# atong01/conditional-flow-matching

Measured on NVIDIA B200. Metric: minibatch-OT couplings/sec (N=8192,d=784), higher is better.
Workload: dtype f32

## Files before the change

cfm_b200/csrc/sinkhorn_common.cuh:

```cuda
#pragma once
#include <cooperative_groups.h>

#include "common.cuh"

namespace cg = cooperative_groups;

namespace cfm {

constexpr int kSkThreads = 512;
constexpr int kSkWarps = kSkThreads / 32;
constexpr int kSkChunk = kSkWarps;
constexpr int kSkMaxKG = 4;
constexpr int kPanelCols = kSkThreads * 4 * kSkMaxKG;

struct SkParams {
  const float* M;
  int n0, n1;
  int64_t ldm;
  float reg;
  const float* cost_max;
  int normalize;
  int max_iters;
  double stop_thr;
  int check_every;
  int precise;
  double stall_tol;
  double* log_u;
  double* log_v;
  int32_t* status;
  double* err_out;
  void* u_work;
  void* v_work[2];
  void* part_m;
  void* part_s;
  double* err_ring;
  int n1p;
  int vec;
  int v_in_smem;
  float l2_resident_frac;
  int dbg_flags;
  int atomic_cols;
  int prefetch_chunks;
  int run_if;
  int timeline;
  int screen_fused;
  int screen;
  int mixed;
};

template <bool P> struct Tr;
template <> struct Tr<false> {
  using pot_t = float;
  using sum_t = float;
  __device__ static __forceinline__ float init() { return -1.0e30f; }
};
template <> struct Tr<true> {
  using pot_t = double;
  using sum_t = double;
  __device__ static __forceinline__ double init() { return -1.0e300; }
};

template <bool P> struct Xf;
template <> struct Xf<false> {
  float c2;
  __device__ __forceinline__ float operator()(float m, float p) const { return fmaf(m, c2, p); }
};
template <> struct Xf<true> {
  float reg, cmax;
  int norm;
  __device__ __forceinline__ double operator()(float m, double p) const {
    const float mn = norm ? __fdiv_rn(m, cmax) : m;
    return (double)(-__fdiv_rn(mn, reg)) + p;
  }
};
__device__ __forceinline__ float expdiff(float x, float m) { return ex2f(x - m); }
__device__ __forceinline__ double expdiff(double x, double m) { return exp(x - m); }
template <bool MIX> __device__ __forceinline__ float expd(float x, float m) { return ex2f(x - m); }
template <bool MIX> __device__ __forceinline__ double expd(double x, double m) {
  if (MIX) return (double)ex2f((float)(x - m) * kLog2e);
  return exp(x - m);
}
__device__ __forceinline__ float lse_fin(float m, float s) { return m + log2f(s); }
__device__ __forceinline__ double lse_fin(double m, double s) { return m + log(s); }
__device__ __forceinline__ float vmax(float a, float b) { return fmaxf(a, b); }
__device__ __forceinline__ double vmax(double a, double b) { return fmax(a, b); }

template <bool VEC>
__device__ __forceinline__ float4 load_cost4(const float* __restrict__ row, int j, int n1) {
  if (VEC) return ldg_stream4(row + j);
  float4 r;
  const float inf = __int_as_float(0x7f800000);
  r.x = (j + 0 < n1) ? __ldg(row + j + 0) : inf;
  r.y = (j + 1 < n1) ? __ldg(row + j + 1) : inf;
  r.z = (j + 2 < n1) ? __ldg(row + j + 2) : inf;
  r.w = (j + 3 < n1) ? __ldg(row + j + 3) : inf;
  return r;
}

template <class T> struct Vec4 { T x, y, z, w; };

template <bool SM, class T>
__device__ __forceinline__ Vec4<T> load_pot4(const T* p, int j) {
  Vec4<T> r;
  if (SM) { r.x = p[j]; r.y = p[j + 1]; r.z = p[j + 2]; r.w = p[j + 3]; }
  else { r.x = __ldcg(p + j); r.y = __ldcg(p + j + 1); r.z = __ldcg(p + j + 2); r.w = __ldcg(p + j + 3); }
  return r;
}

}
```

cfm_b200/csrc/sinkhorn_v2.cu:

```cuda
#include <stdlib.h>

#include "sinkhorn_common.cuh"

namespace cfm {


__device__ __forceinline__ uint32_t v2_smem_u32(const void* p) { return (uint32_t)__cvta_generic_to_shared(p); }
__device__ __forceinline__ void v2_mbar_init(uint64_t* bar, uint32_t count) {
  asm volatile("mbarrier.init.shared::cta.b64 [%0], %1;" ::"r"(v2_smem_u32(bar)), "r"(count));
}
__device__ __forceinline__ void v2_mbar_expect_tx(uint64_t* bar, uint32_t bytes) {
  asm volatile("mbarrier.arrive.expect_tx.shared::cta.b64 _, [%0], %1;" ::"r"(v2_smem_u32(bar)), "r"(bytes) : "memory");
}
__device__ __forceinline__ void v2_mbar_arrive(uint64_t* bar) {
  asm volatile("mbarrier.arrive.shared::cta.b64 _, [%0];" ::"r"(v2_smem_u32(bar)) : "memory");
}
__device__ __forceinline__ void v2_mbar_wait(uint64_t* bar, uint32_t parity) {
  asm volatile(
      "{\n\t"
      ".reg .pred p;\n\t"
      "WAIT_%=:\n\t"
      "mbarrier.try_wait.parity.shared::cta.b64 p, [%0], %1;\n\t"
      "@p bra DONE_%=;\n\t"
      "bra WAIT_%=;\n\t"
      "DONE_%=:\n\t"
      "}\n" ::"r"(v2_smem_u32(bar)), "r"(parity) : "memory");
}
__device__ __forceinline__ void v2_bulk_load(void* dst, const void* src, uint32_t bytes, uint64_t* bar) {
  asm volatile("cp.async.bulk.shared::cluster.global.mbarrier::complete_tx::bytes [%0], [%1], %2, [%3];"
               ::"r"(v2_smem_u32(dst)), "l"(src), "r"(bytes), "r"(v2_smem_u32(bar)) : "memory");
}
__device__ __forceinline__ void v2_bulk_load_hint(void* dst, const void* src, uint32_t bytes, uint64_t* bar,
                                                  uint64_t policy) {
  asm volatile("cp.async.bulk.shared::cluster.global.mbarrier::complete_tx::bytes.L2::cache_hint [%0], [%1], %2, [%3], %4;"
               ::"r"(v2_smem_u32(dst)), "l"(src), "r"(bytes), "r"(v2_smem_u32(bar)), "l"(policy) : "memory");
}
__device__ __forceinline__ void v2_prefetch_l2(const void* src, uint32_t bytes) {
  asm volatile("cp.async.bulk.prefetch.L2.global [%0], %1;" ::"l"(src), "r"(bytes) : "memory");
}
__device__ __forceinline__ uint64_t v2_policy_evict_last() {
  uint64_t p;
  asm volatile("createpolicy.fractional.L2::evict_last.b64 %0, 1.0;" : "=l"(p));
  return p;
}
__device__ __forceinline__ uint64_t v2_policy_evict_first() {
  uint64_t p;
  asm volatile("createpolicy.fractional.L2::evict_first.b64 %0, 1.0;" : "=l"(p));
  return p;
}
__device__ __forceinline__ void v2_grid_barrier(unsigned int* counter, unsigned int target) {
  __syncthreads();
  if (threadIdx.x == 0) {
    __threadfence();
    atomicAdd(counter, 1u);
    unsigned int seen;
    do {
      asm volatile("ld.acquire.gpu.global.u32 %0, [%1];" : "=r"(seen) : "l"(counter) : "memory");
    } while (seen < target);
    __threadfence();
  }
  __syncthreads();
}
template <int NT>
__device__ __forceinline__ void v2_consumer_barrier() { asm volatile("bar.sync 1, %0;" ::"n"(NT) : "memory"); }

template <int R>
__device__ __forceinline__ void multi_reduce(float (&v)[R], int lane) {
  static_assert(R == 1 || R == 2 || R == 4 || R == 8, "R must be a power of two <= 8");
  int off = 16;
#pragma unroll
  for (int n = R; n > 1; n >>= 1) {
    const bool upper = (lane & off) != 0;
#pragma unroll
    for (int i = 0; i < n / 2; ++i) {
      const float a = v[2 * i], b = v[2 * i + 1];
      const float send = upper ? a : b, keep = upper ? b : a;
      v[i] = keep + __shfl_xor_sync(0xffffffffu, send, off);
    }
    off >>= 1;
  }
  for (; off > 0; off >>= 1) v[0] += __shfl_xor_sync(0xffffffffu, v[0], off);
}
template <int R>
__device__ __forceinline__ int multi_row(int lane) {
  int r = 0, bit = 4;
#pragma unroll
  for (int n = R, sh = 0; n > 1; n >>= 1, ++sh, --bit) r |= ((lane >> bit) & 1) << sh;
  return r;
}

template <int NT, int KG, int R>
__global__ void __launch_bounds__(NT, 512 / NT) sinkhorn_v2_kernel(const SkParams p, const int S) {
  constexpr int kV2Consumers = NT, kV2Threads = NT, kV2Warps = NT / 32;
  constexpr bool kVSmem = KG > 4;
  extern __shared__ __align__(128) unsigned char v2_smem[];
  cg::grid_group grid = cg::this_grid();
  const int tid = threadIdx.x, lane = tid & 31, warp = tid >> 5;
  const int nblk = gridDim.x, b = blockIdx.x;
  const int n0 = p.n0, n1 = p.n1, n1p = p.n1p, ng = n1p / 4;

  if (p.run_if != 0) {
    const float cmax = p.cost_max ? __ldg(p.cost_max) : 0.f;
    const bool precise = !((p.normalize ? 1.f : cmax) / p.reg <= 64.f);
    if (precise) return;
  }

  const uint32_t stage_floats = (uint32_t)R * (uint32_t)n1p;
  float* stages = reinterpret_cast<float*>(v2_smem);
  float2* rowpart = reinterpret_cast<float2*>(stages + (size_t)S * stage_floats);
  uint64_t* full = reinterpret_cast<uint64_t*>(rowpart + 2 * R * kV2Warps);
  float* V_s = reinterpret_cast<float*>(full + 8);
  __shared__ double red[kV2Warps];

  if (tid == 0) {
    for (int s = 0; s < S; ++s) v2_mbar_init(&full[s], 1);
    asm volatile("fence.mbarrier_init.release.cluster;" ::: "memory");
  }
  __syncthreads();

  float* u_work = reinterpret_cast<float*>(p.u_work);
  float* v_work[2] = {reinterpret_cast<float*>(p.v_work[0]), reinterpret_cast<float*>(p.v_work[1])};
  float* part_m = reinterpret_cast<float*>(p.part_m);
  float* part_s = reinterpret_cast<float*>(p.part_s);

  const float cmaxv = p.cost_max ? __ldg(p.cost_max) : 1.f;
  const float c2 = -kLog2e / (p.reg * (p.normalize ? cmaxv : 1.f));
  const float loga = -log2f((float)n0), logb = -log2f((float)n1);
  const float kappa = c2 * cmaxv;
  const bool fact = (p.cost_max != nullptr) && (-kappa <= 40.f);

  const int base = n0 / nblk, rem = n0 % nblk;
  const int r_begin = b * base + min(b, rem);
  const int nrows = base + (b < rem ? 1 : 0);
  const int nchunks = (nrows + R - 1) / R;

  int c_st = 0;
  uint32_t c_par = 0;
  int p_st = 0, p_chunk = 0;
  int p_dir = 1;
  int sweep_no = 0;
  unsigned int* gbar = reinterpret_cast<unsigned int*>(p.err_ring + 4);
  unsigned int gbar_n = 0;
  auto grid_sync = [&]() { (void)gbar; (void)gbar_n; grid.sync(); };
  long long issued = 0, consumed_total = 0;
  bool gvalid[KG];
#pragma unroll
  for (int k = 0; k < KG; ++k) gvalid[k] = (tid + kV2Consumers * k) < ng;
  const int tcol = tid * 4;
  const bool full_cols = ng == kV2Consumers * KG;

  const int resident = p.l2_resident_frac > 0.f ? (int)(p.l2_resident_frac * (float)nchunks) : -1;
  const uint64_t pol_last = v2_policy_evict_last(), pol_first = v2_policy_evict_first();
  auto issue_next = [&]() {
    const int r0 = r_begin + p_chunk * R;
    const int rv = min(R, r_begin + nrows - r0);
    v2_mbar_expect_tx(&full[p_st], (uint32_t)rv * (uint32_t)n1 * 4u);
    for (int r = 0; r < rv; ++r) {
      float* dst = stages + (size_t)p_st * stage_floats + (size_t)r * n1p;
      const float* src = p.M + (int64_t)(r0 + r) * p.ldm;
      if (resident < 0) v2_bulk_load(dst, src, (uint32_t)n1 * 4u, &full[p_st]);
      else v2_bulk_load_hint(dst, src, (uint32_t)n1 * 4u, &full[p_st], p_chunk < resident ? pol_last : pol_first);
    }
    ++issued;
    p_chunk += p_dir;
    if (p_chunk == nchunks) { p_chunk = nchunks - 1; p_dir = -1; }
    else if (p_chunk < 0) { p_chunk = 0; p_dir = 1; }
    if (++p_st == S) p_st = 0;
  };
  if (tid == 0)
    for (int q = 0; q < S; ++q) issue_next();
  auto prefetch_ahead = [&]() {
    int c = p_chunk, dir = p_dir;
    for (int q = 0; q < p.prefetch_chunks; ++q) {
      if (c < 0 || c >= nchunks) break;
      if (!(resident >= 0 && c < resident)) {
        const int r0 = r_begin + c * R;
        const int rv = min(R, r_begin + nrows - r0);
        for (int r = 0; r < rv; ++r) v2_prefetch_l2(p.M + (int64_t)(r0 + r) * p.ldm, (uint32_t)n1 * 4u);
      }
      c += dir;
    }
  };

  auto sweep = [&](bool do_row, bool do_col, const float* v_cur, const float4* v_in, float vref_in,
                   unsigned long long* acc_out, const float* v_reload) {
    if (fact) {
      const float vref = do_row ? (v_in ? vref_in : __ldcg(v_cur)) : 0.f;
      const float nkap = -kappa;
      float4 V[kVSmem ? 1 : KG];
      float cs[KG][4];
#pragma unroll
      for (int k = 0; k < KG; ++k) {
        float4 vk = make_float4(0.f, 0.f, 0.f, 0.f);
        if (gvalid[k]) {
          if (do_row) {
            const float4 vv = v_in ? v_in[k]
                                   : __ldcg(reinterpret_cast<const float4*>(v_cur + tcol + kV2Consumers * 4 * k));
            vk = make_float4(ex2f(vv.x - vref), ex2f(vv.y - vref), ex2f(vv.z - vref), ex2f(vv.w - vref));
          } else {
            vk = make_float4(1.f, 1.f, 1.f, 1.f);
          }
        }
        if (kVSmem) *reinterpret_cast<float4*>(V_s + tcol + kV2Consumers * 4 * k) = vk;
        else V[k] = vk;
#pragma unroll
        for (int c = 0; c < 4; ++c) cs[k][c] = 0.f;
      }
      float uref = 0.f;
      bool have_uref = !do_row;
      for (int cc = 0; cc < nchunks; ++cc) {
        const int chunk = (sweep_no & 1) ? nchunks - 1 - cc : cc;
        const int r0 = r_begin + chunk * R;
        const int rv = min(R, r_begin + nrows - r0);
        const float* sbase = stages + (uint32_t)c_st * stage_floats + tcol;
        float2* rp = rowpart + (cc & 1) * R * kV2Warps;
        v2_mbar_wait(&full[c_st], c_par);
        float4 E[R][KG];
        if (full_cols && rv == R) {
#pragma unroll
          for (int r = 0; r < R; ++r)
#pragma unroll
            for (int k = 0; k < KG; ++k) {
              const float4 mv = *reinterpret_cast<const float4*>(sbase + r * n1p + kV2Consumers * 4 * k);
              E[r][k] = make_float4(ex2f(fmaf(mv.x, c2, nkap)), ex2f(fmaf(mv.y, c2, nkap)),
                                    ex2f(fmaf(mv.z, c2, nkap)), ex2f(fmaf(mv.w, c2, nkap)));
            }
        } else {
#pragma unroll
          for (int r = 0; r < R; ++r) {
            const float* srow = sbase + r * n1p;
#pragma unroll
            for (int k = 0; k < KG; ++k) {
              E[r][k] = make_float4(0.f, 0.f, 0.f, 0.f);
              if (gvalid[k] && r < rv) {
                const float4 mv = *reinterpret_cast<const float4*>(srow + kV2Consumers * 4 * k);
                E[r][k] = make_float4(ex2f(fmaf(mv.x, c2, nkap)), ex2f(fmaf(mv.y, c2, nkap)),
                                      ex2f(fmaf(mv.z, c2, nkap)), ex2f(fmaf(mv.w, c2, nkap)));
              }
            }
          }
        }
        if (++c_st == S) { c_st = 0; c_par ^= 1u; }
        if (do_row) {
          float sr[R];
#pragma unroll
          for (int r = 0; r < R; ++r) {
            float s = 0.f;
#pragma unroll
            for (int k = 0; k < KG; ++k) {
              const float4 vk = kVSmem ? *reinterpret_cast<const float4*>(V_s + tcol + kV2Consumers * 4 * k)
                                       : V[kVSmem ? 0 : k];
              s = fmaf(E[r][k].x, vk.x, s); s = fmaf(E[r][k].y, vk.y, s);
              s = fmaf(E[r][k].z, vk.z, s); s = fmaf(E[r][k].w, vk.w, s);
            }
            sr[r] = s;
          }
          multi_reduce<R>(sr, lane);
          if ((lane & (32 / R - 1)) == 0) rp[multi_row<R>(lane) * kV2Warps + warp] = make_float2(sr[0], 0.f);
        }
        v2_consumer_barrier<NT>();
        if (tid == 0) issue_next();
        float U[R];
        if (do_row) {
#pragma unroll
          for (int rr = 0; rr < R; rr += 2) {
            const int myrow = rr + (lane >> 4);
            float pr = ((R == 1 && lane >= 16) || (lane & 15) >= kV2Warps)
                           ? 0.f : rp[(R == 1 ? 0 : myrow) * kV2Warps + (lane & 15)].x;
#pragma unroll
            for (int o = 8; o > 0; o >>= 1) pr += __shfl_xor_sync(0xffffffffu, pr, o);
            float Srow[2];
            Srow[0] = __shfl_sync(0xffffffffu, pr, 0);
            Srow[1] = __shfl_sync(0xffffffffu, pr, 16);
#pragma unroll
            for (int h = 0; h < 2; ++h) {
              const int r = rr + h;
              if (r < R) {
                const float u2 = loga - (kappa + vref + lg2_abs(Srow[h]));
                if (!have_uref) { uref = u2; have_uref = true; }
                U[r] = r < rv ? ex2f(u2 - uref) : 0.f;
                if (warp == 0 && lane == 0 && r < rv) {
                  u_work[r0 + r] = u2;
                  p.log_u[r0 + r] = (double)u2 * kLn2d;
                }
              }
            }
          }
        } else {
#pragma unroll
          for (int r = 0; r < R; ++r) U[r] = 1.f;
        }
        if (do_col) {
#pragma unroll
          for (int r = 0; r < R; ++r)
#pragma unroll
            for (int k = 0; k < KG; ++k) {
              cs[k][0] = fmaf(E[r][k].x, U[r], cs[k][0]); cs[k][1] = fmaf(E[r][k].y, U[r], cs[k][1]);
              cs[k][2] = fmaf(E[r][k].z, U[r], cs[k][2]); cs[k][3] = fmaf(E[r][k].w, U[r], cs[k][3]);
            }
        }
      }
      consumed_total += nchunks;
      ++sweep_no;
      if (tid == 0) prefetch_ahead();
      if (do_col && acc_out != nullptr) {
        const float sh = kappa + uref - logb;
#pragma unroll
        for (int k = 0; k < KG; ++k)
          if (gvalid[k]) {
            const float4 vv = v_reload ? __ldcg(reinterpret_cast<const float4*>(v_reload + tcol + kV2Consumers * 4 * k))
                                       : make_float4(0.f, 0.f, 0.f, 0.f);
            const float vq[4] = {vv.x, vv.y, vv.z, vv.w};
            unsigned long long* dst = acc_out + tcol + kV2Consumers * 4 * k;
#pragma unroll
            for (int c = 0; c < 4; ++c) {
              const float q = cs[k][c] * ex2f(sh + vq[c]) * 4294967296.f;
              atomicAdd(dst + c, (unsigned long long)__float2ll_rn(fminf(fmaxf(q, 0.f), 4.0e18f)));
            }
          }
      } else if (do_col) {
        const float pm = kappa + uref;
#pragma unroll
        for (int k = 0; k < KG; ++k)
          if (gvalid[k]) {
            *reinterpret_cast<float4*>(part_m + (int64_t)b * n1p + tcol + kV2Consumers * 4 * k) =
                make_float4(pm, pm, pm, pm);
            *reinterpret_cast<float4*>(part_s + (int64_t)b * n1p + tcol + kV2Consumers * 4 * k) =
                make_float4(cs[k][0], cs[k][1], cs[k][2], cs[k][3]);
          }
      }
      return;
    }
    float4 vreg[KG];
    float cm[KG][4], cs[KG][4];
#pragma unroll
    for (int k = 0; k < KG; ++k) {
      vreg[k] = make_float4(0.f, 0.f, 0.f, 0.f);
      if (do_row && gvalid[k]) {
        const float* vp = v_cur + tcol + kV2Consumers * 4 * k;
        vreg[k] = make_float4(__ldcg(vp), __ldcg(vp + 1), __ldcg(vp + 2), __ldcg(vp + 3));
      }
#pragma unroll
      for (int c = 0; c < 4; ++c) { cm[k][c] = -1.0e30f; cs[k][c] = 0.f; }
    }
    const float inf = __int_as_float(0x7f800000);
    for (int cc = 0; cc < nchunks; ++cc) {
      const int chunk = (sweep_no & 1) ? nchunks - 1 - cc : cc;
      const int r0 = r_begin + chunk * R;
      const int rv = min(R, r_begin + nrows - r0);
      const float* sbase = stages + (uint32_t)c_st * stage_floats + tcol;
      float2* rp = rowpart + (cc & 1) * R * kV2Warps;
      v2_mbar_wait(&full[c_st], c_par);
      if (++c_st == S) { c_st = 0; c_par ^= 1u; }
      float u2[R];
      if (do_row) {
#pragma unroll
        for (int r = 0; r < R; ++r) {
          float x[KG][4];
          float tmax = -1.0e30f;
#pragma unroll
          for (int k = 0; k < KG; ++k) {
            float4 mv = make_float4(inf, inf, inf, inf);
            if (gvalid[k] && r < rv) mv = *reinterpret_cast<const float4*>(sbase + r * n1p + kV2Consumers * 4 * k);
            x[k][0] = fmaf(mv.x, c2, vreg[k].x); x[k][1] = fmaf(mv.y, c2, vreg[k].y);
            x[k][2] = fmaf(mv.z, c2, vreg[k].z); x[k][3] = fmaf(mv.w, c2, vreg[k].w);
            tmax = fmaxf(tmax, fmaxf(fmaxf(x[k][0], x[k][1]), fmaxf(x[k][2], x[k][3])));
          }
          const float wm = warp_max(tmax);
          float s = 0.f;
#pragma unroll
          for (int k = 0; k < KG; ++k)
            s += (ex2f(x[k][0] - wm) + ex2f(x[k][1] - wm)) + (ex2f(x[k][2] - wm) + ex2f(x[k][3] - wm));
          s = warp_sum(s);
          if (lane == 0) rp[r * kV2Warps + warp] = make_float2(wm, s);
        }
      }
      v2_consumer_barrier<NT>();
#pragma unroll
      for (int r = 0; r < R; ++r) {
        u2[r] = 0.f;
        if (do_row) {
          const float2 pr = lane < kV2Warps ? rp[r * kV2Warps + lane] : make_float2(-1.0e30f, 0.f);
          const float gm = warp_max(pr.x);
          const float gs = warp_sum(pr.y * ex2f(pr.x - gm));
          u2[r] = loga - (gm + log2f(gs));
          if (warp == 0 && lane == 0 && r < rv) {
            u_work[r0 + r] = u2[r];
            p.log_u[r0 + r] = (double)u2[r] * kLn2d;
          }
        }
      }
      if (do_col) {
#pragma unroll
        for (int r = 0; r < R; ++r) {
          if (r < rv) {
#pragma unroll
            for (int k = 0; k < KG; ++k) {
              if (gvalid[k]) {
                const float4 mv = *reinterpret_cast<const float4*>(sbase + r * n1p + kV2Consumers * 4 * k);
                const float xv[4] = {fmaf(mv.x, c2, u2[r]), fmaf(mv.y, c2, u2[r]), fmaf(mv.z, c2, u2[r]),
                                     fmaf(mv.w, c2, u2[r])};
#pragma unroll
                for (int c = 0; c < 4; ++c) {
                  if (xv[c] > cm[k][c] + 40.f) {
                    cs[k][c] *= ex2f(cm[k][c] - xv[c]);
                    cm[k][c] = xv[c];
                  }
                  cs[k][c] += ex2f(xv[c] - cm[k][c]);
                }
              }
            }
          }
        }
      }
      v2_consumer_barrier<NT>();
      if (tid == 0) issue_next();
    }
    consumed_total += nchunks;
    ++sweep_no;
    if (tid == 0) prefetch_ahead();
    if (do_col) {
#pragma unroll
      for (int k = 0; k < KG; ++k)
        if (gvalid[k]) {
          *reinterpret_cast<float4*>(part_m + (int64_t)b * n1p + tcol + kV2Consumers * 4 * k) =
              make_float4(cm[k][0], cm[k][1], cm[k][2], cm[k][3]);
          *reinterpret_cast<float4*>(part_s + (int64_t)b * n1p + tcol + kV2Consumers * 4 * k) =
              make_float4(cs[k][0], cs[k][1], cs[k][2], cs[k][3]);
        }
    }
  };

  auto combine = [&](const float* v_cur, float* v_new, bool have_cur, double* err_slot) {
    double err_local = 0.0;
    const int cpc = (n1 + nblk - 1) / nblk;
    const int c_begin = b * cpc, c_end = min(n1, c_begin + cpc);
    const int sub = tid & 7;
    for (int j0 = c_begin; j0 < c_end; j0 += (kV2Consumers >> 3)) {
      const int j = j0 + (tid >> 3);
      const bool act = j < c_end;
      float m = -1.0e30f, s = 0.f;
      if (act) {
        if (p.dbg_flags & 1) {
          for (int c0 = sub; c0 < nblk; c0 += 32) {
            float mm[4], ss[4];
#pragma unroll
            for (int q = 0; q < 4; ++q) {
              const int c = c0 + q * 8;
              if (c < nblk) {
                mm[q] = __ldcg(part_m + (int64_t)c * n1p + j);
                ss[q] = __ldcg(part_s + (int64_t)c * n1p + j);
              } else { mm[q] = -1.0e30f; ss[q] = 0.f; }
            }
            const float bm = fmaxf(fmaxf(fmaxf(mm[0], mm[1]), fmaxf(mm[2], mm[3])), m);
            float acc = s * ex2f(m - bm);
#pragma unroll
            for (int q = 0; q < 4; ++q) acc += ss[q] * ex2f(mm[q] - bm);
            s = acc; m = bm;
          }
        } else if (!(p.dbg_flags & 4) && nblk <= 152) {
          float mm[19], ss[19];
#pragma unroll
          for (int q = 0; q < 19; ++q) {
            const int c = sub + q * 8;
            if (c < nblk) {
              mm[q] = __ldcg(part_m + (int64_t)c * n1p + j);
              ss[q] = __ldcg(part_s + (int64_t)c * n1p + j);
            } else { mm[q] = -1.0e30f; ss[q] = 0.f; }
          }
          float bm = m;
#pragma unroll
          for (int q = 0; q < 19; ++q) bm = fmaxf(bm, mm[q]);
          float acc = 0.f;
#pragma unroll
          for (int q = 0; q < 19; ++q) acc += ss[q] * ex2f(mm[q] - bm);
          s = acc; m = bm;
        } else
        for (int c0 = sub; c0 < nblk; c0 += 64) {
          float mm[8], ss[8];
#pragma unroll
          for (int q = 0; q < 8; ++q) {
            const int c = c0 + q * 8;
            if (c < nblk) {
              mm[q] = __ldcg(part_m + (int64_t)c * n1p + j);
              ss[q] = __ldcg(part_s + (int64_t)c * n1p + j);
            } else { mm[q] = -1.0e30f; ss[q] = 0.f; }
          }
          float bm = m;
#pragma unroll
          for (int q = 0; q < 8; ++q) bm = fmaxf(bm, mm[q]);
          float acc = s * ex2f(m - bm);
#pragma unroll
          for (int q = 0; q < 8; ++q) acc += ss[q] * ex2f(mm[q] - bm);
          s = acc; m = bm;
        }
      }
      float gm = m;
#pragma unroll
      for (int o = 4; o > 0; o >>= 1) gm = fmaxf(gm, __shfl_xor_sync(0xffffffffu, gm, o));
      float gs = s * ex2f(m - gm);
#pragma unroll
      for (int o = 4; o > 0; o >>= 1) gs += __shfl_xor_sync(0xffffffffu, gs, o);
      if (act && sub == 0) {
        const float vn = logb - (gm + log2f(gs));
        v_new[j] = vn;
        if (have_cur) {
          const double d = ((double)__ldcg(v_cur + j) - (double)vn) * kLn2d;
          const double e = expm1(d) / (double)n1;
          err_local += e * e;
        }
      }
    }
    if (err_slot != nullptr) {
      err_local = warp_sum(err_local);
      if (lane == 0) red[warp] = err_local;
      __syncthreads();
      if (warp == 0) {
        double t = lane < kV2Warps ? red[lane] : 0.0;
        t = warp_sum(t);
        if (lane == 0) atomicAdd(err_slot, t);
      }
      __syncthreads();
    }
  };

  if (b == 0 && tid < 4) p.err_ring[tid] = 0.0;

  int cur = 0, iters = 0;
  bool converged = false;
  double err = 1.0, prev_check_err = -1.0;
  const bool single = fact && p.atomic_cols != 0;
  if (single) {
    unsigned long long* acc = reinterpret_cast<unsigned long long*>(p.part_s);
    float* vmine = part_m + (int64_t)b * n1p;
#pragma unroll
    for (int k = 0; k < KG; ++k)
      if (gvalid[k]) *reinterpret_cast<float4*>(vmine + tcol + kV2Consumers * 4 * k) = make_float4(0.f, 0.f, 0.f, 0.f);
    float vref_cur = 0.f;
    const int cpc = ((n1 + nblk - 1) / nblk + 3) & ~3;
    sweep(false, true, nullptr, nullptr, 0.f, acc, nullptr);
    grid_sync();
    for (int it = 0;; ++it) {
      const unsigned long long* tot = acc + (size_t)(it % 3) * n1p;
      {
        unsigned long long* z = acc + (size_t)((it + 2) % 3) * n1p;
        for (int j = b * cpc + tid; j < min(n1, (b + 1) * cpc); j += kV2Threads) z[j] = 0ull;
      }
      float4 vnew[KG];
      double e2 = 0.0;
      const float t0 = (float)((double)__ldcg(tot) * 2.3283064365386963e-10);
      const float vref_new = vref_cur - lg2_abs(t0);
#pragma unroll
      for (int k = 0; k < KG; ++k) {
        float4 vcur_k = make_float4(0.f, 0.f, 0.f, 0.f);
        if (gvalid[k]) vcur_k = __ldcg(reinterpret_cast<const float4*>(vmine + tcol + kV2Consumers * 4 * k));
        vnew[k] = vcur_k;
        if (gvalid[k]) {
          const ulonglong2 a = __ldcg(reinterpret_cast<const ulonglong2*>(tot + tcol + kV2Consumers * 4 * k));
          const ulonglong2 c = __ldcg(reinterpret_cast<const ulonglong2*>(tot + tcol + kV2Consumers * 4 * k + 2));
          const double td[4] = {(double)a.x * 2.3283064365386963e-10, (double)a.y * 2.3283064365386963e-10,
                                (double)c.x * 2.3283064365386963e-10, (double)c.y * 2.3283064365386963e-10};
          vnew[k] = make_float4(vcur_k.x - lg2_abs((float)td[0]), vcur_k.y - lg2_abs((float)td[1]),
                                vcur_k.z - lg2_abs((float)td[2]), vcur_k.w - lg2_abs((float)td[3]));
#pragma unroll
          for (int q = 0; q < 4; ++q) e2 += (td[q] - 1.0) * (td[q] - 1.0);
        }
      }
      if (it >= 1 && (((it - 1) % p.check_every) == 0 || (p.dbg_flags & 2))) {
        e2 = warp_sum(e2);
        if (lane == 0) red[warp] = e2;
        __syncthreads();
        double t = 0.0;
        for (int w = 0; w < kV2Warps; ++w) t += red[w];
        __syncthreads();
        err = sqrt(t) / (double)n1;
        if (((it - 1) % p.check_every) == 0) {
          if (err < p.stop_thr) { converged = true; break; }
          if (p.stall_tol > 0.0 && prev_check_err >= 0.0 && err > (1.0 - p.stall_tol) * prev_check_err &&
              err * sqrt((double)n1) < 1e-5) { converged = true; break; }
          prev_check_err = err;
        }
      }
      if (it == p.max_iters) break;
#pragma unroll
      for (int k = 0; k < KG; ++k)
        if (gvalid[k]) *reinterpret_cast<float4*>(vmine + tcol + kV2Consumers * 4 * k) = vnew[k];
      vref_cur = vref_new;
      const bool last = (it == p.max_iters - 1);
      const bool check = (it % p.check_every) == 0;
      const bool do_col = !last || check;
      sweep(true, do_col, nullptr, vnew, vref_cur, do_col ? acc + (size_t)((it + 1) % 3) * n1p : nullptr, vmine);
      iters = it + 1;
      if (!do_col) break;
      grid_sync();
    }
    if (b == 0) {
#pragma unroll
      for (int k = 0; k < KG; ++k)
        if (gvalid[k]) {
          const int j = tcol + kV2Consumers * 4 * k;
          const float4 vv = __ldcg(reinterpret_cast<const float4*>(vmine + j));
          p.log_v[j] = (double)vv.x * kLn2d; p.log_v[j + 1] = (double)vv.y * kLn2d;
          p.log_v[j + 2] = (double)vv.z * kLn2d; p.log_v[j + 3] = (double)vv.w * kLn2d;
        }
    }
  } else {
  sweep(false, true, nullptr, nullptr, 0.f, nullptr, nullptr);
  grid_sync();
  combine(nullptr, v_work[0], false, nullptr);
  grid_sync();

  for (int it = 0; it < p.max_iters; ++it) {
    const bool last = (it == p.max_iters - 1);
    const bool check = (it % p.check_every) == 0;
    const bool do_col = !last || check;
    sweep(true, do_col, v_work[cur], nullptr, 0.f, nullptr, nullptr);
    iters = it + 1;
    if (!do_col) break;
    grid_sync();
    if (b == 0 && tid == 0) p.err_ring[(it + 2) & 3] = 0.0;
    const bool want_err = check || (p.dbg_flags & 2);
    combine(v_work[cur], v_work[cur ^ 1], want_err, want_err ? &p.err_ring[it & 3] : nullptr);
    grid_sync();
    if (check) {
      err = sqrt(__ldcg(&p.err_ring[it & 3]));
      if (err < p.stop_thr) { converged = true; break; }
      if (p.stall_tol > 0.0 && prev_check_err >= 0.0 && err > (1.0 - p.stall_tol) * prev_check_err &&
          err * sqrt((double)n1) < 1e-5) { converged = true; break; }
      prev_check_err = err;
    }
    if (last) break;
    cur ^= 1;
  }
  }

  if (tid == 0) {
    for (long long q = consumed_total; q < issued; ++q) {
      v2_mbar_wait(&full[c_st], c_par);
      if (++c_st == S) { c_st = 0; c_par ^= 1u; }
    }
  }

  if (!single)
    for (int j = b * kV2Threads + tid; j < n1; j += nblk * kV2Threads)
      p.log_v[j] = (double)__ldcg(v_work[cur] + j) * kLn2d;
  if (b == 0 && tid == 0) {
    int flags = 0;
    if (!converged) flags |= CFM_FLAG_NOT_CONVERGED;
    if (!(err == err)) flags |= CFM_FLAG_NONFINITE;
    p.status[0] = flags;
    p.status[1] = iters;
    p.status[2] = 0;
    p.status[3] = fact ? (single ? 4 : 3) : 2;
    *p.err_out = err;
  }
}

template <int NT, int KG, int R>
static int v2_launch_t(SkParams& p, cudaStream_t s) {
  auto kern = sinkhorn_v2_kernel<NT, KG, R>;
  constexpr int kPerSm = 512 / NT;
  const size_t stage_bytes = (size_t)R * p.n1p * 4;
  const size_t fixed = (size_t)2 * R * (NT / 32) * sizeof(float2) + 8 * sizeof(uint64_t) + 128 +
                       (KG > 4 ? (size_t)p.n1p * 4 : 0);
  const size_t budget = (kPerSm == 1 ? 220 : 108) * 1024;
  if (budget < fixed + 2 * stage_bytes) return 1;
  int S = (int)((budget - fixed) / stage_bytes);
  if (S > 8) S = 8;
  const size_t smem = (size_t)S * stage_bytes + fixed;
  CFM_CUDA_OK(cudaFuncSetAttribute(kern, cudaFuncAttributeMaxDynamicSharedMemorySize, (int)smem));
  int per_sm = 0;
  CFM_CUDA_OK(cudaOccupancyMaxActiveBlocksPerMultiprocessor(&per_sm, kern, NT, smem));
  if (per_sm < 1) return 1;
  if (per_sm > kPerSm) per_sm = kPerSm;
  int grid = sm_count() * per_sm;
  if (grid > p.n0) grid = p.n0;
  void* args[] = {(void*)&p, (void*)&S};
  CFM_CUDA_OK(cudaMemsetAsync(p.err_ring + 4, 0, 16, s));
  if (p.atomic_cols)
    CFM_CUDA_OK(cudaMemsetAsync(p.part_s, 0, (size_t)3 * p.n1p * sizeof(unsigned long long), s));
  CFM_CUDA_OK(cudaLaunchCooperativeKernel((void*)kern, dim3(grid), dim3(NT), args, smem, s));
  note_launches(1);
  return CFM_OK;
}

int sinkhorn_v2_launch(SkParams& p, cudaStream_t s) {
  if (!p.vec || p.n1p > 8192 || p.n1p != p.n1) return 1;
  static float l2frac = -2.f;
  if (l2frac < -1.f) { const char* e = getenv("CFM_SK_L2"); l2frac = e ? (float)atof(e) : 0.15f; }
  p.l2_resident_frac = ((size_t)p.n0 * p.n1 * 4 > (size_t)100 << 20) ? l2frac : 0.f;
  static int dbg = -1;
  if (dbg < 0) { const char* e = getenv("CFM_SK_DBG"); dbg = e ? atoi(e) : 0; }
  p.dbg_flags = dbg;
  static int pf = -1;
  if (pf < 0) { const char* e = getenv("CFM_SK_PF"); pf = e ? atoi(e) : 0; }
  p.prefetch_chunks = ((size_t)p.n0 * p.n1 * 4 > (size_t)100 << 20) ? pf : 0;
  static int atom = -1;
  if (atom < 0) { const char* e = getenv("CFM_SK_ATOMIC"); atom = e ? atoi(e) : 0; }
  p.atomic_cols = atom;
  static long persist = -2;
  if (persist == -2) {
    const char* e = getenv("CFM_SK_PERSIST_MB");
    persist = e ? atol(e) : -1;
    if (persist >= 0) cudaDeviceSetLimit(cudaLimitPersistingL2CacheSize, (size_t)persist << 20);
  }
  static int cfg = -1;
  if (cfg < 0) { const char* e = getenv("CFM_SK_CONFIG"); cfg = e ? atoi(e) : 0; }
  const int ng = p.n1p / 4;
#ifdef CFM_SK_BUILD_256
  if (cfg == 2) {
    const int kg = (ng + 255) / 256;
    int rc = 1;
    if (kg <= 1) rc = v2_launch_t<256, 1, 8>(p, s);
    else if (kg <= 2) rc = v2_launch_t<256, 2, 4>(p, s);
    else if (kg <= 4) rc = v2_launch_t<256, 4, 2>(p, s);
    else rc = v2_launch_t<256, 8, 1>(p, s);
    if (rc != 1) return rc;
  }
#endif
  const int kg = (ng + 511) / 512;
  if (kg <= 1) return v2_launch_t<512, 1, 8>(p, s);
  if (kg <= 2) return v2_launch_t<512, 2, 4>(p, s);
  return v2_launch_t<512, 4, 2>(p, s);
}

}
```

Baseline: 203.7.

## Cache up to four exponentiated cost chunks per block in Blackwell tensor memory

Allocates TMEM per CTA and, on the first sweep, stores the exp-transformed cost tiles of up to four chosen chunks into it. Later Sinkhorn sweeps read those chunks back from TMEM and skip both the bulk global loads and the exponentials, and the producer's issue order is changed to step over them. This cuts L2/HBM traffic and SFU work per iteration. In exchange it adds TMEM alloc/ld/st with synchronous waits and more complex producer/consumer bookkeeping, which could break pipeline balance.

After: 177.9 (median of 6 runs). 12.6% lower.

```diff
diff --git a/cfm_b200/csrc/sinkhorn_common.cuh b/cfm_b200/csrc/sinkhorn_common.cuh
--- a/cfm_b200/csrc/sinkhorn_common.cuh
+++ b/cfm_b200/csrc/sinkhorn_common.cuh
@@ -41,6 +41,7 @@
   int dbg_flags;
   int atomic_cols;
   int prefetch_chunks;
+  int tmem_chunks;
   int run_if;
   int timeline;
   int screen_fused;
diff --git a/cfm_b200/csrc/sinkhorn_v2.cu b/cfm_b200/csrc/sinkhorn_v2.cu
--- a/cfm_b200/csrc/sinkhorn_v2.cu
+++ b/cfm_b200/csrc/sinkhorn_v2.cu
@@ -48,6 +48,57 @@
   asm volatile("createpolicy.fractional.L2::evict_first.b64 %0, 1.0;" : "=l"(p));
   return p;
 }
+__device__ __forceinline__ void v2_tmem_alloc(uint32_t* dst_smem, uint32_t ncols) {
+  asm volatile("tcgen05.alloc.cta_group::1.sync.aligned.shared::cta.b32 [%0], %1;" ::"r"(v2_smem_u32(dst_smem)),
+               "r"(ncols) : "memory");
+  asm volatile("tcgen05.relinquish_alloc_permit.cta_group::1.sync.aligned;" ::: "memory");
+}
+__device__ __forceinline__ void v2_tmem_dealloc(uint32_t base, uint32_t ncols) {
+  asm volatile("tcgen05.dealloc.cta_group::1.sync.aligned.b32 %0, %1;" ::"r"(base), "r"(ncols) : "memory");
+}
+__device__ __forceinline__ void v2_tmem_fence_before() { asm volatile("tcgen05.fence::before_thread_sync;" ::: "memory"); }
+__device__ __forceinline__ void v2_tmem_fence_after() { asm volatile("tcgen05.fence::after_thread_sync;" ::: "memory"); }
+template <int R, int KG>
+__device__ __forceinline__ void v2_tmem_st32(uint32_t taddr, const float4 (&E)[R][KG]) {
+  static_assert(R * KG == 8, "one chunk of one thread = 32 floats = one .x32 slot");
+  uint32_t v[32];
+#pragma unroll
+  for (int i = 0; i < 8; ++i) {
+    const float4 e = E[i / KG][i % KG];
+    v[4 * i] = __float_as_uint(e.x); v[4 * i + 1] = __float_as_uint(e.y);
+    v[4 * i + 2] = __float_as_uint(e.z); v[4 * i + 3] = __float_as_uint(e.w);
+  }
+  asm volatile(
+      "tcgen05.st.sync.aligned.32x32b.x32.b32 [%0], "
+      "{%1, %2, %3, %4, %5, %6, %7, %8, %9, %10, %11, %12, %13, %14, %15, %16, "
+      "%17, %18, %19, %20, %21, %22, %23, %24, %25, %26, %27, %28, %29, %30, %31, %32};\n\t"
+      "tcgen05.wait::st.sync.aligned;"
+      ::"r"(taddr), "r"(v[0]), "r"(v[1]), "r"(v[2]), "r"(v[3]), "r"(v[4]), "r"(v[5]), "r"(v[6]), "r"(v[7]),
+        "r"(v[8]), "r"(v[9]), "r"(v[10]), "r"(v[11]), "r"(v[12]), "r"(v[13]), "r"(v[14]), "r"(v[15]),
+        "r"(v[16]), "r"(v[17]), "r"(v[18]), "r"(v[19]), "r"(v[20]), "r"(v[21]), "r"(v[22]), "r"(v[23]),
+        "r"(v[24]), "r"(v[25]), "r"(v[26]), "r"(v[27]), "r"(v[28]), "r"(v[29]), "r"(v[30]), "r"(v[31])
+      : "memory");
+}
+template <int R, int KG>
+__device__ __forceinline__ void v2_tmem_ld32(uint32_t taddr, float4 (&E)[R][KG]) {
+  static_assert(R * KG == 8, "one chunk of one thread = 32 floats = one .x32 slot");
+  uint32_t v[32];
+  asm volatile(
+      "tcgen05.ld.sync.aligned.32x32b.x32.b32 "
+      "{%0, %1, %2, %3, %4, %5, %6, %7, %8, %9, %10, %11, %12, %13, %14, %15, "
+      "%16, %17, %18, %19, %20, %21, %22, %23, %24, %25, %26, %27, %28, %29, %30, %31}, [%32];\n\t"
+      "tcgen05.wait::ld.sync.aligned;"
+      : "=r"(v[0]), "=r"(v[1]), "=r"(v[2]), "=r"(v[3]), "=r"(v[4]), "=r"(v[5]), "=r"(v[6]), "=r"(v[7]),
+        "=r"(v[8]), "=r"(v[9]), "=r"(v[10]), "=r"(v[11]), "=r"(v[12]), "=r"(v[13]), "=r"(v[14]), "=r"(v[15]),
+        "=r"(v[16]), "=r"(v[17]), "=r"(v[18]), "=r"(v[19]), "=r"(v[20]), "=r"(v[21]), "=r"(v[22]), "=r"(v[23]),
+        "=r"(v[24]), "=r"(v[25]), "=r"(v[26]), "=r"(v[27]), "=r"(v[28]), "=r"(v[29]), "=r"(v[30]), "=r"(v[31])
+      : "r"(taddr)
+      : "memory");
+#pragma unroll
+  for (int i = 0; i < 8; ++i)
+    E[i / KG][i % KG] = make_float4(__uint_as_float(v[4 * i]), __uint_as_float(v[4 * i + 1]),
+                                    __uint_as_float(v[4 * i + 2]), __uint_as_float(v[4 * i + 3]));
+}
 __device__ __forceinline__ void v2_grid_barrier(unsigned int* counter, unsigned int target) {
   __syncthreads();
   if (threadIdx.x == 0) {
@@ -111,12 +162,8 @@
   uint64_t* full = reinterpret_cast<uint64_t*>(rowpart + 2 * R * kV2Warps);
   float* V_s = reinterpret_cast<float*>(full + 8);
   __shared__ double red[kV2Warps];
-
-  if (tid == 0) {
-    for (int s = 0; s < S; ++s) v2_mbar_init(&full[s], 1);
-    asm volatile("fence.mbarrier_init.release.cluster;" ::: "memory");
-  }
-  __syncthreads();
+  __shared__ uint32_t tm_base_s;
+  __shared__ int4 tm_pos_s;
 
   float* u_work = reinterpret_cast<float*>(p.u_work);
   float* v_work[2] = {reinterpret_cast<float*>(p.v_work[0]), reinterpret_cast<float*>(p.v_work[1])};
@@ -133,6 +180,36 @@
   const int r_begin = b * base + min(b, rem);
   const int nrows = base + (b < rem ? 1 : 0);
   const int nchunks = (nrows + R - 1) / R;
+  const int resident = p.l2_resident_frac > 0.f ? (int)(p.l2_resident_frac * (float)nchunks) : -1;
+
+  static_assert(R * KG == 8, "TMEM slot = the 32 floats one thread holds of one chunk");
+  const int tm_n = fact ? min(min(max(p.tmem_chunks, 0), 4), nchunks) : 0;
+  const int tm_stream = nchunks - tm_n;
+
+  if (tid == 0) {
+    for (int s = 0; s < S; ++s) v2_mbar_init(&full[s], 1);
+    asm volatile("fence.mbarrier_init.release.cluster;" ::: "memory");
+    const int margin = nchunks / 8;
+    int lo = max(resident, 0) + margin, hi = nchunks - margin;
+    if (hi - lo < tm_n) { lo = (nchunks - tm_n) / 2; hi = lo + tm_n; }
+    if (p.dbg_flags & 8) { lo += (hi - lo - tm_n) / 2; hi = lo + tm_n; }
+    int pos[4];
+#pragma unroll
+    for (int s = 0; s < 4; ++s) pos[s] = s < tm_n ? lo + ((2 * s + 1) * (hi - lo)) / (2 * tm_n) : -1;
+    tm_pos_s = make_int4(pos[0], pos[1], pos[2], pos[3]);
+  }
+  if (tm_n > 0 && warp == 0) {
+    __syncwarp();
+    v2_tmem_alloc(&tm_base_s, (uint32_t)NT);
+  }
+  v2_tmem_fence_before();
+  __syncthreads();
+  v2_tmem_fence_after();
+  const uint32_t tm_addr = tm_n > 0 ? tm_base_s + ((uint32_t)(32 * (warp & 3)) << 16) + (uint32_t)(128 * (warp >> 2)) : 0u;
+  auto tm_slot = [&](int chunk) -> int {
+    const int4 tp = tm_pos_s;
+    return chunk == tp.x ? 0 : chunk == tp.y ? 1 : chunk == tp.z ? 2 : chunk == tp.w ? 3 : -1;
+  };
 
   int c_st = 0;
   uint32_t c_par = 0;
@@ -149,9 +226,10 @@
   const int tcol = tid * 4;
   const bool full_cols = ng == kV2Consumers * KG;
 
-  const int resident = p.l2_resident_frac > 0.f ? (int)(p.l2_resident_frac * (float)nchunks) : -1;
+  bool p_skip_tm = false;
   const uint64_t pol_last = v2_policy_evict_last(), pol_first = v2_policy_evict_first();
   auto issue_next = [&]() {
+    if (p_skip_tm && tm_stream == 0) return;
     const int r0 = r_begin + p_chunk * R;
     const int rv = min(R, r_begin + nrows - r0);
     v2_mbar_expect_tx(&full[p_st], (uint32_t)rv * (uint32_t)n1 * 4u);
@@ -162,9 +240,11 @@
       else v2_bulk_load_hint(dst, src, (uint32_t)n1 * 4u, &full[p_st], p_chunk < resident ? pol_last : pol_first);
     }
     ++issued;
-    p_chunk += p_dir;
-    if (p_chunk == nchunks) { p_chunk = nchunks - 1; p_dir = -1; }
-    else if (p_chunk < 0) { p_chunk = 0; p_dir = 1; }
+    do {
+      p_chunk += p_dir;
+      if (p_chunk == nchunks) { p_chunk = nchunks - 1; p_dir = -1; p_skip_tm = tm_n > 0; }
+      else if (p_chunk < 0) { p_chunk = 0; p_dir = 1; }
+    } while (p_skip_tm && tm_stream > 0 && tm_slot(p_chunk) >= 0);
     if (++p_st == S) p_st = 0;
   };
   if (tid == 0)
@@ -173,7 +253,7 @@
     int c = p_chunk, dir = p_dir;
     for (int q = 0; q < p.prefetch_chunks; ++q) {
       if (c < 0 || c >= nchunks) break;
-      if (!(resident >= 0 && c < resident)) {
+      if (!(resident >= 0 && c < resident) && tm_slot(c) < 0) {
         const int r0 = r_begin + c * R;
         const int rv = min(R, r_begin + nrows - r0);
         for (int r = 0; r < rv; ++r) v2_prefetch_l2(p.M + (int64_t)(r0 + r) * p.ldm, (uint32_t)n1 * 4u);
@@ -214,33 +294,40 @@
         const int rv = min(R, r_begin + nrows - r0);
         const float* sbase = stages + (uint32_t)c_st * stage_floats + tcol;
         float2* rp = rowpart + (cc & 1) * R * kV2Warps;
-        v2_mbar_wait(&full[c_st], c_par);
+        const int slot = tm_n > 0 ? tm_slot(chunk) : -1;
+        const bool from_tm = slot >= 0 && sweep_no > 0;
         float4 E[R][KG];
-        if (full_cols && rv == R) {
-#pragma unroll
-          for (int r = 0; r < R; ++r)
-#pragma unroll
-            for (int k = 0; k < KG; ++k) {
-              const float4 mv = *reinterpret_cast<const float4*>(sbase + r * n1p + kV2Consumers * 4 * k);
-              E[r][k] = make_float4(ex2f(fmaf(mv.x, c2, nkap)), ex2f(fmaf(mv.y, c2, nkap)),
-                                    ex2f(fmaf(mv.z, c2, nkap)), ex2f(fmaf(mv.w, c2, nkap)));
-            }
+        if (from_tm) {
+          v2_tmem_ld32<R, KG>(tm_addr + 32u * (uint32_t)slot, E);
         } else {
-#pragma unroll
-          for (int r = 0; r < R; ++r) {
-            const float* srow = sbase + r * n1p;
-#pragma unroll
-            for (int k = 0; k < KG; ++k) {
-              E[r][k] = make_float4(0.f, 0.f, 0.f, 0.f);
-              if (gvalid[k] && r < rv) {
-                const float4 mv = *reinterpret_cast<const float4*>(srow + kV2Consumers * 4 * k);
+          v2_mbar_wait(&full[c_st], c_par);
+          if (full_cols && rv == R) {
+#pragma unroll
+            for (int r = 0; r < R; ++r)
+#pragma unroll
+              for (int k = 0; k < KG; ++k) {
+                const float4 mv = *reinterpret_cast<const float4*>(sbase + r * n1p + kV2Consumers * 4 * k);
                 E[r][k] = make_float4(ex2f(fmaf(mv.x, c2, nkap)), ex2f(fmaf(mv.y, c2, nkap)),
                                       ex2f(fmaf(mv.z, c2, nkap)), ex2f(fmaf(mv.w, c2, nkap)));
               }
+          } else {
+#pragma unroll
+            for (int r = 0; r < R; ++r) {
+              const float* srow = sbase + r * n1p;
+#pragma unroll
+              for (int k = 0; k < KG; ++k) {
+                E[r][k] = make_float4(0.f, 0.f, 0.f, 0.f);
+                if (gvalid[k] && r < rv) {
+                  const float4 mv = *reinterpret_cast<const float4*>(srow + kV2Consumers * 4 * k);
+                  E[r][k] = make_float4(ex2f(fmaf(mv.x, c2, nkap)), ex2f(fmaf(mv.y, c2, nkap)),
+                                        ex2f(fmaf(mv.z, c2, nkap)), ex2f(fmaf(mv.w, c2, nkap)));
+                }
+              }
             }
           }
-        }
-        if (++c_st == S) { c_st = 0; c_par ^= 1u; }
+          if (++c_st == S) { c_st = 0; c_par ^= 1u; }
+          if (slot >= 0) v2_tmem_st32<R, KG>(tm_addr + 32u * (uint32_t)slot, E);
+        }
         if (do_row) {
           float sr[R];
 #pragma unroll
@@ -259,7 +346,7 @@
           if ((lane & (32 / R - 1)) == 0) rp[multi_row<R>(lane) * kV2Warps + warp] = make_float2(sr[0], 0.f);
         }
         v2_consumer_barrier<NT>();
-        if (tid == 0) issue_next();
+        if (tid == 0 && !from_tm) issue_next();
         float U[R];
         if (do_row) {
 #pragma unroll
@@ -300,7 +387,7 @@
             }
         }
       }
-      consumed_total += nchunks;
+      consumed_total += sweep_no == 0 ? nchunks : tm_stream;
       ++sweep_no;
       if (tid == 0) prefetch_ahead();
       if (do_col && acc_out != nullptr) {
@@ -638,6 +725,14 @@
     for (long long q = consumed_total; q < issued; ++q) {
       v2_mbar_wait(&full[c_st], c_par);
       if (++c_st == S) { c_st = 0; c_par ^= 1u; }
+    }
+  }
+  if (tm_n > 0) {
+    v2_tmem_fence_before();
+    __syncthreads();
+    if (warp == 0) {
+      v2_tmem_fence_after();
+      v2_tmem_dealloc(tm_base_s, (uint32_t)NT);
     }
   }
 
@@ -698,6 +793,9 @@
   static int atom = -1;
   if (atom < 0) { const char* e = getenv("CFM_SK_ATOMIC"); atom = e ? atoi(e) : 0; }
   p.atomic_cols = atom;
+  static int tmem = -1;
+  if (tmem < 0) { const char* e = getenv("CFM_SK_TMEM"); tmem = e ? min(max(atoi(e), 0), 4) : 4; }
+  p.tmem_chunks = tmem;
   static long persist = -2;
   if (persist == -2) {
     const char* e = getenv("CFM_SK_PERSIST_MB");
```
